# RazonIn4K/image-restoration-platform

Measured on AMD Instinct MI355X. Metric: restored images/sec @1024x1024 bs=8, higher is better.
Workload: dtype bf16; 1 GPU; 1024x1024 RGB u8, batch 8 per GPU: fused classifier scan + RestoreNet-v0 (43 convs, 779.9 GFLOP/image), seeded random-init weights; global_batch=8, parallelism=per-image data parallel x1, no collective, streams=1

## Files before the change

### image_restoration_platform_amd/csrc/conv_up.hip

```cpp
#include "conv_mfma.hpp"
#include "persist.hpp"

#include <type_traits>

namespace ire {

namespace {

typedef __bf16 bf16x8_t __attribute__((ext_vector_type(8)));
typedef __bf16 bf16x2_t __attribute__((ext_vector_type(2)));
typedef float f32x2_t __attribute__((ext_vector_type(2)));
typedef float f32x16_t __attribute__((ext_vector_type(16)));
typedef unsigned u32x4_t __attribute__((ext_vector_type(4)));

#ifndef IRE_UP_TEPI
#define IRE_UP_TEPI 1
#endif
#ifndef IRE_UP_ABL
#define IRE_UP_ABL 0
#endif
constexpr int UP_THREADS = 512;
constexpr int UP_TH = 16, UP_TW = 32;
constexpr int UP_IH = UP_TH + 2, UP_IW = UP_TW + 2;
constexpr int UP_IN_CHUNKS = UP_IH * UP_IW * 4;
constexpr int UP_IN_ITERS = (UP_IN_CHUNKS + UP_THREADS - 1) / UP_THREADS;
constexpr int UP_IN_BYTES = UP_IN_ITERS * UP_THREADS * 16;
constexpr int UP_NT = 32;
constexpr int UP_W_CHUNKS = 4 * 16 * UP_NT;
constexpr int UP_W_BYTES = UP_W_CHUNKS * 16;
constexpr int UP_W_ITERS = UP_W_CHUNKS / UP_THREADS;
constexpr int UP_BUF = UP_IN_BYTES + UP_W_BYTES;
constexpr int UP_BIAS_OFF = 2 * UP_BUF;
constexpr int UP_SKW_OFF = UP_BIAS_OFF + 256 * 4;
constexpr int UP_RED_OFF = UP_SKW_OFF + 8192;
constexpr int UP_LDS = UP_RED_OFF + 8 * 8 * 2 * 4;
static_assert(UP_LDS <= 160 * 1024, "LDS");
constexpr int UP_PATCH = UP_BUF / 8;

__device__ __forceinline__ unsigned up_pack(float a, float b) {
    f32x2_t f = {a, b};
    return __builtin_bit_cast(unsigned, __builtin_convertvector(f, bf16x2_t));
}
__device__ __forceinline__ void up_glds16(const void* gsrc, unsigned lds_dst_uniform) {
    unsigned keep;
    asm volatile("s_mov_b32 %0, m0\n\ts_mov_b32 m0, %2\n\ts_nop 0\n\tglobal_load_lds_dwordx4 %1, off\n\ts_mov_b32 m0, %0"
                 : "=&s"(keep) : "v"(gsrc), "s"(lds_dst_uniform) : "memory");
}

template <int N> __device__ __forceinline__ float up_ror_add(float v) {
    const int r = __builtin_amdgcn_update_dpp(0, __builtin_bit_cast(int, v), 0x120 + N, 0xf, 0xf, false);
    return v + __builtin_bit_cast(float, r);
}
__device__ __forceinline__ float up_swap16_add(float v) {
    float x = v, y = v;
    asm volatile("v_nop\n\tv_nop\n\tv_permlane16_swap_b32 %0, %1" : "+v"(x), "+v"(y));
    return x + y;
}

template <int I, int N, class F> __device__ __forceinline__ void up_static_for(F& f) {
    if constexpr (I < N) { f(std::integral_constant<int, I>{}); up_static_for<I + 1, N>(f); }
}

using UpItem = PersistItem;
struct UpRegs { uint4 v[UP_IN_ITERS]; };

template <int NKS>
__global__ __launch_bounds__(UP_THREADS) void conv_up_kernel(ConvArgs a) {
    __shared__ __attribute__((aligned(16))) unsigned char smem[UP_LDS];
    const unsigned smem_lds = (unsigned)(size_t)(__attribute__((address_space(3))) unsigned char*)smem;
    const int tid = threadIdx.x;
    const int lane = tid & 63, wave = tid >> 6;
    const int r = lane & 31, h = lane >> 5;
    const int c8_fixed = tid & 3;

    PersistCursor cursor(a.tiles_x, a.tiles_y, a.nimg, a.nblocks, a.nkc, (int)gridDim.x, (int)blockIdx.x, a.walk_rev != 0);
    const int my_items = cursor.my_items;
    const int nkc = a.nkc;
    const int S = cursor.S;
    if (S == 0) return;
    using StageInfo = PersistStage;
    StageInfo sq0 = cursor.cur, sq1 = cursor.next(), sq2 = cursor.next();

    const int Cin = a.cin0;
    const int cin_shift = 31 - __builtin_clz(Cin);

    int a_off[2][9];
#pragma unroll
    for (int m = 0; m < 2; ++m)
#pragma unroll
        for (int tap = 0; tap < 9; ++tap) {
            const int ky = tap / 3, kx = tap - ky * 3;
            const int p = (wave * 2 + m + ky) * UP_IW + r + kx;
            a_off[m][tap] = (p * 4 + (h ^ ((p >> 2) & 3))) * 16;
        }
    const int b_off = (h * UP_NT + r) * 16;

    auto load_chunk = [&](const StageInfo& si, int i, UpRegs& R) {
        const UpItem& it = si.it;
        const int oy1 = it.ty * UP_TH - 1, ox1 = it.tx * UP_TW - 1;
        const char* base = reinterpret_cast<const char*>(a.in0) + (size_t)it.img * a.in_rows * a.Win * Cin * 2 + si.kc * 64;
        const __amdgpu_buffer_rsrc_t irsrc = __builtin_amdgcn_make_buffer_rsrc(const_cast<char*>(base), 0, a.in_rows * a.Win * Cin * 2 - si.kc * 64, 0x00020000);
        int t2 = tid;
        asm volatile("" : "+v"(t2));
        const int p = (t2 + i * UP_THREADS) >> 2;
        const int py = p / UP_IW, px = p - py * UP_IW;
        const int iy = oy1 + py, ix = ox1 + px;
        const bool ok = (unsigned)(iy - a.iy_lo) < (unsigned)a.iy_span && (unsigned)ix < (unsigned)a.Win;
        const unsigned off = ok ? ((unsigned)((iy + a.in_row_off) * a.Win + ix) << (cin_shift + 1)) + (unsigned)(c8_fixed * 16) : 0xffffffffu;
        const u32x4_t lv = __builtin_amdgcn_raw_buffer_load_b128(irsrc, off, 0, 0);
        R.v[i] = make_uint4(lv.x, lv.y, lv.z, lv.w);
    };
    auto load_stage = [&](const StageInfo& si, UpRegs& R) {
#pragma unroll
        for (int i = 0; i < UP_IN_ITERS; ++i) load_chunk(si, i, R);
    };
    auto store_chunk = [&](int i, const UpRegs& R, uint4* lds_in) {
        int t2 = tid;
        asm volatile("" : "+v"(t2));
        const int idx = t2 + i * UP_THREADS;
        const int p = idx >> 2;
        lds_in[p * 4 + (c8_fixed ^ ((p >> 2) & 3))] = R.v[i];
    };
    auto wslab = [&](const StageInfo& si) -> const unsigned char* {
        return reinterpret_cast<const unsigned char*>(a.w) + ((size_t)si.it.nb * nkc + si.kc) * UP_W_BYTES;
    };

    f32x16_t acc[4][2];
    const float* bias_lds = reinterpret_cast<const float*>(smem + UP_BIAS_OFF);
    const int tiles_per_img = a.tiles_x * a.tiles_y;
    UpRegs R;

    auto epilogue = [&](const UpItem& it) __attribute__((always_inline)) {
        int r_e = r, h_e = h, w_e = wave;
        asm volatile("" : "+v"(r_e), "+v"(h_e), "+v"(w_e));
        char* obase = reinterpret_cast<char*>(a.out) + (size_t)it.img * a.Hout * a.Wout * a.cout * 2;
        const __amdgpu_buffer_rsrc_t orsrc = __builtin_amdgcn_make_buffer_rsrc(obase, 0, a.Hout * a.Wout * a.cout * 2, 0x00020000);
        const int ly = it.ty * UP_TH + w_e * 2, lx = it.tx * UP_TW + r_e;
        if constexpr (NKS > 0) {
            constexpr int NKG = NKS / 2;
            constexpr int U = 8 * NKG;
#ifdef IRE_UP_D
            constexpr int D = IRE_UP_D;
#else
            constexpr int D = NKS <= 2 ? 4 : NKS == 4 ? 3 : 2;
#endif
            const int C = a.cout;
            const char* sbase = reinterpret_cast<const char*>(a.in1) + (size_t)it.img * a.Hout * a.Wout * C * 2;
            const __amdgpu_buffer_rsrc_t srsrc = __builtin_amdgcn_make_buffer_rsrc(const_cast<char*>(sbase), 0, a.Hout * a.Wout * C * 2, 0x00020000);
            const unsigned rowB = (unsigned)(a.Wout * C * 2), pxB = (unsigned)(C * 2);
            const unsigned s_off = (unsigned)((2 * ly) * a.Wout + 2 * lx) * pxB + (unsigned)(h_e * 16);
            const bool inb[2] = {ly < a.Hin && lx < a.Win, ly + 1 < a.Hin && lx < a.Win};
            const unsigned char* skw = smem + UP_SKW_OFF + (h_e * 32 + r_e) * 16;
            const bf16x2_t ones = __builtin_bit_cast(bf16x2_t, 0x3f803f80u);
            u32x4_t ring[D][2];
            float ssum[4] = {0.f, 0.f, 0.f, 0.f}, qsum[4] = {0.f, 0.f, 0.f, 0.f};
            auto issue = [&](auto u_tag) __attribute__((always_inline)) {
                constexpr int u = decltype(u_tag)::value;
                constexpr int pm = u / NKG, kg = u % NKG, par = pm >> 1, m = pm & 1, pa = par >> 1, pb = par & 1;
                const unsigned off = s_off + (unsigned)(2 * m + pa) * rowB + (unsigned)pb * pxB + (unsigned)(kg * 64);
                ring[u % D][0] = __builtin_amdgcn_raw_buffer_load_b128(srsrc, off, 0, 0);
                ring[u % D][1] = __builtin_amdgcn_raw_buffer_load_b128(srsrc, off + 32u, 0, 0);
            };
            auto consume = [&](auto u_tag) __attribute__((always_inline)) {
                constexpr int u = decltype(u_tag)::value;
                constexpr int pm = u / NKG, kg = u % NKG, par = pm >> 1, m = pm & 1;
                const bf16x8_t w0 = __builtin_bit_cast(bf16x8_t, *reinterpret_cast<const uint4*>(skw + (2 * kg) * 1024));
                const bf16x8_t w1 = __builtin_bit_cast(bf16x8_t, *reinterpret_cast<const uint4*>(skw + (2 * kg + 1) * 1024));
                acc[par][m] = __builtin_amdgcn_mfma_f32_32x32x16_bf16(w0, __builtin_bit_cast(bf16x8_t, ring[u % D][0]), acc[par][m], 0, 0, 0);
                acc[par][m] = __builtin_amdgcn_mfma_f32_32x32x16_bf16(w1, __builtin_bit_cast(bf16x8_t, ring[u % D][1]), acc[par][m], 0, 0, 0);
            };
            auto finish = [&](auto par_tag) __attribute__((always_inline)) {
                constexpr int par = decltype(par_tag)::value;
                constexpr int pa = par >> 1, pb = par & 1;
                const int ox = 2 * lx + pb;
#pragma unroll
                for (int m = 0; m < 2; ++m) {
                    const int oy = 2 * (ly + m) + pa;
                    const unsigned off = ((unsigned)((oy * a.Wout + ox) * a.cout + it.nb * UP_NT) << 1) + (unsigned)(h_e * 16);
                    const f32x16_t& c = acc[par][m];
#pragma unroll
                    for (int pp = 0; pp < 2; ++pp) {
                        unsigned w[4] = {up_pack(c[8 * pp + 0], c[8 * pp + 1]), up_pack(c[8 * pp + 2], c[8 * pp + 3]),
                                         up_pack(c[8 * pp + 4], c[8 * pp + 5]), up_pack(c[8 * pp + 6], c[8 * pp + 7])};
                        const u32x4_t wv4 = {w[0], w[1], w[2], w[3]};
                        if constexpr (!(IRE_UP_ABL & 4)) __builtin_amdgcn_raw_buffer_store_b128(wv4, orsrc, inb[m] ? off + (unsigned)(pp * 32) : 0xffffffffu, 0, IRE_ST_PART);
                        else asm volatile("" :: "v"(wv4));
                        if constexpr (!(IRE_UP_ABL & 2))
#pragma unroll
                        for (int d = 0; d < 4; ++d) {
                            const bf16x2_t wv = __builtin_bit_cast(bf16x2_t, inb[m] ? w[d] : 0u);
                            ssum[2 * pp + (d >> 1)] = __builtin_amdgcn_fdot2_f32_bf16(wv, ones, ssum[2 * pp + (d >> 1)], false);
                            qsum[2 * pp + (d >> 1)] = __builtin_amdgcn_fdot2_f32_bf16(wv, wv, qsum[2 * pp + (d >> 1)], false);
                        }
                    }
                }
            };
            auto unit = [&](auto u_tag) __attribute__((always_inline)) {
                constexpr int u = decltype(u_tag)::value;
                if constexpr (!(IRE_UP_ABL & 1)) {
                consume(u_tag);
                if constexpr (u + D < U) issue(std::integral_constant<int, u + D>{});
                }
                if constexpr ((u + 1) % (2 * NKG) == 0) finish(std::integral_constant<int, u / (2 * NKG)>{});
            };
            if constexpr (!(IRE_UP_ABL & 1)) up_static_for<0, D>(issue);
            up_static_for<0, U>(unit);
            if constexpr (!(IRE_UP_ABL & 2)) {
            float rv[8] = {ssum[0], qsum[0], ssum[1], qsum[1], ssum[2], qsum[2], ssum[3], qsum[3]};
#pragma unroll
            for (int i = 0; i < 8; ++i) rv[i] = up_ror_add<1>(rv[i]);
#pragma unroll
            for (int i = 0; i < 8; ++i) rv[i] = up_ror_add<2>(rv[i]);
#pragma unroll
            for (int i = 0; i < 8; ++i) rv[i] = up_ror_add<4>(rv[i]);
#pragma unroll
            for (int i = 0; i < 8; ++i) rv[i] = up_ror_add<8>(rv[i]);
#pragma unroll
            for (int i = 0; i < 8; ++i) rv[i] = up_swap16_add(rv[i]);
            float* red = reinterpret_cast<float*>(smem + UP_RED_OFF);
            if (r_e == 0) {
#pragma unroll
                for (int k = 0; k < 4; ++k)
                    *reinterpret_cast<float2*>(red + (w_e * 8 + (k >> 1) * 4 + 2 * h_e + (k & 1)) * 2) = make_float2(rv[2 * k], rv[2 * k + 1]);
            }
            __syncthreads();
            const int G = a.group_size, qpg = G >> 2, ngl = UP_NT / G;
            if (tid < ngl) {
                float sv = 0.f, qv = 0.f;
#pragma unroll
                for (int w = 0; w < 8; ++w)
#pragma unroll
                    for (int k = 0; k < 4; ++k)
                        if (k < qpg) { sv += red[(w * 8 + tid * qpg + k) * 2 + 0]; qv += red[(w * 8 + tid * qpg + k) * 2 + 1]; }
                float* st = a.stats + (((size_t)it.img * tiles_per_img + it.tile) * 8 + (it.nb * UP_NT) / G + tid) * 2;
                st[0] = sv; st[1] = qv;
            }
            }
        } else {
#pragma unroll
        for (int par = 0; par < 4; ++par) {
            const int pa = par >> 1, pb = par & 1;
            const int ox = 2 * lx + pb;
#pragma unroll
            for (int m = 0; m < 2; ++m) {
                const int oy = 2 * (ly + m) + pa;
                const bool inb = oy < a.Hout && ox < a.Wout;
                const unsigned off = ((unsigned)((oy * a.Wout + ox) * a.cout + it.nb * UP_NT) << 1) + (unsigned)(h_e * 16);
                const f32x16_t& c = acc[par][m];
#pragma unroll
                for (int pp = 0; pp < 2; ++pp) {
                    const u32x4_t wv4 = {up_pack(c[8 * pp + 0], c[8 * pp + 1]), up_pack(c[8 * pp + 2], c[8 * pp + 3]),
                                         up_pack(c[8 * pp + 4], c[8 * pp + 5]), up_pack(c[8 * pp + 6], c[8 * pp + 7])};
                    __builtin_amdgcn_raw_buffer_store_b128(wv4, orsrc, inb ? off + (unsigned)(pp * 32) : 0xffffffffu, 0, IRE_ST_PART);
                }
            }
        }
        }
#pragma unroll
        for (int par = 0; par < 4; ++par)
#pragma unroll
            for (int m = 0; m < 2; ++m) asm volatile("" : "=v"(acc[par][m]));
    };

    u32x4_t skpre[4];
    auto epi_prefetch = [&](const UpItem& it) __attribute__((always_inline)) {
        constexpr int C = 16 * (NKS > 0 ? NKS : 2);
        int l_e = lane, w_e = wave;
        asm volatile("" : "+v"(l_e), "+v"(w_e));
        const char* sbase = reinterpret_cast<const char*>(a.in1) + (size_t)it.img * a.Hout * a.Wout * C * 2;
        const __amdgpu_buffer_rsrc_t srsrc = __builtin_amdgcn_make_buffer_rsrc(const_cast<char*>(sbase), 0, a.Hout * a.Wout * C * 2, 0x00020000);
        const int ly = it.ty * UP_TH + w_e * 2, ox0 = 2 * it.tx * UP_TW;
        const int lc = l_e & 3, lp0 = l_e >> 2;
        const bool rowok = ly < a.Hin;
#pragma unroll
        for (int i = 0; i < 4; ++i) {
            const int p = lp0 + i * 16;
            const bool ok = rowok && ox0 + p < a.Wout;
            skpre[i] = __builtin_amdgcn_raw_buffer_load_b128(srsrc, ok ? (unsigned)((((2 * ly) * a.Wout + ox0 + p) * C + lc * 8) * 2) : 0xffffffffu, 0, C == 32 ? IRE_LD_ONCE : 0);
        }
    };
    auto epilogue_t = [&](const UpItem& it) __attribute__((always_inline)) {
        constexpr int C = 16 * (NKS > 0 ? NKS : 2);
        constexpr int PCH = 32;
        constexpr int NPIECE = C / PCH;
        constexpr int CPP = PCH / 8;
        constexpr int KSP = PCH / 16;
        constexpr int PSTEP = 64 / CPP;
        int l_e = lane, w_e = wave;
        asm volatile("" : "+v"(l_e), "+v"(w_e));
        const int r_e = l_e & 31, h_e = l_e >> 5;
        unsigned char* patch = smem + UP_BUF + w_e * UP_PATCH;
        char* obase = reinterpret_cast<char*>(a.out) + (size_t)it.img * a.Hout * a.Wout * C * 2;
        const __amdgpu_buffer_rsrc_t orsrc = __builtin_amdgcn_make_buffer_rsrc(obase, 0, a.Hout * a.Wout * C * 2, 0x00020000);
        const char* sbase = reinterpret_cast<const char*>(a.in1) + (size_t)it.img * a.Hout * a.Wout * C * 2;
        const __amdgpu_buffer_rsrc_t srsrc = __builtin_amdgcn_make_buffer_rsrc(const_cast<char*>(sbase), 0, a.Hout * a.Wout * C * 2, 0x00020000);
        const int ly = it.ty * UP_TH + w_e * 2, ox0 = 2 * it.tx * UP_TW;
        const unsigned char* skw = smem + UP_SKW_OFF + (h_e * 32 + r_e) * 16;
        const bf16x2_t ones = __builtin_bit_cast(bf16x2_t, 0x3f803f80u);
        const int lc = l_e % CPP, lp0 = l_e / CPP;
        const unsigned ld_lds = (unsigned)(lp0 * (CPP * 16) + ((lc ^ ((lp0 >> 1) & (CPP - 1))) << 4));
        const int sp0 = l_e >> 2, scq = l_e & 3;
        float ssum[2] = {0.f, 0.f}, qsum[2] = {0.f, 0.f};
        u32x4_t sk[CPP];
        auto issue_piece = [&](int rr, int pc) __attribute__((always_inline)) {
            const int m = rr >> 1, pa = rr & 1;
            const int oy = 2 * (ly + m) + pa;
            const bool rowok = ly + m < a.Hin;
#pragma unroll
            for (int i = 0; i < CPP; ++i) {
                const int p = lp0 + i * PSTEP;
                const bool ok = rowok && ox0 + p < a.Wout;
                sk[i] = __builtin_amdgcn_raw_buffer_load_b128(srsrc, ok ? (unsigned)(((oy * a.Wout + ox0 + p) * C + pc * PCH + lc * 8) * 2) : 0xffffffffu, 0, C == 32 ? IRE_LD_ONCE : 0);
            }
        };
        if constexpr (!(IRE_UP_ABL & 1)) {
#pragma unroll
            for (int i = 0; i < CPP; ++i) sk[i] = skpre[i];
        }
#pragma unroll
        for (int rr = 0; rr < 4; ++rr) {
            const int m = rr >> 1, pa = rr & 1;
            if constexpr (!(IRE_UP_ABL & 1))
#pragma unroll
            for (int pc = 0; pc < NPIECE; ++pc) {
#pragma unroll
                for (int i = 0; i < CPP; ++i) *reinterpret_cast<u32x4_t*>(patch + ld_lds + i * (PSTEP * CPP * 16)) = sk[i];
                if (rr * NPIECE + pc + 1 < 4 * NPIECE) issue_piece((rr * NPIECE + pc + 1) / NPIECE, (rr * NPIECE + pc + 1) % NPIECE);
#pragma unroll
                for (int pb = 0; pb < 2; ++pb)
#pragma unroll
                    for (int k = 0; k < KSP; ++k) {
                        const bf16x8_t wk = __builtin_bit_cast(bf16x8_t, *reinterpret_cast<const uint4*>(skw + (pc * KSP + k) * 1024));
                        const bf16x8_t fr = __builtin_bit_cast(bf16x8_t, *reinterpret_cast<const uint4*>(patch + (2 * r_e + pb) * (CPP * 16) + (((2 * k + h_e) ^ (r_e & (CPP - 1))) << 4)));
                        acc[pa * 2 + pb][m] = __builtin_amdgcn_mfma_f32_32x32x16_bf16(wk, fr, acc[pa * 2 + pb][m], 0, 0, 0);
                    }
            }
            const int oy = 2 * (ly + m) + pa;
            const bool rowok = ly + m < a.Hin;
#pragma unroll
            for (int pb = 0; pb < 2; ++pb) {
                const f32x16_t& c = acc[pa * 2 + pb][m];
#pragma unroll
                for (int pp = 0; pp < 2; ++pp) {
                    const u32x4_t wv = {up_pack(c[8 * pp + 0], c[8 * pp + 1]), up_pack(c[8 * pp + 2], c[8 * pp + 3]),
                                        up_pack(c[8 * pp + 4], c[8 * pp + 5]), up_pack(c[8 * pp + 6], c[8 * pp + 7])};
                    *reinterpret_cast<u32x4_t*>(patch + (2 * r_e + pb) * 64 + (((2 * pp + h_e) ^ (r_e & 3)) << 4)) = wv;
                }
            }
#pragma unroll
            for (int k = 0; k < 4; ++k) {
                const int p = sp0 + 16 * k;
                const u32x4_t v = *reinterpret_cast<const u32x4_t*>(patch + p * 64 + ((scq ^ ((p >> 1) & 3)) << 4));
                const bool ok = rowok && ox0 + p < a.Wout;
                const unsigned w[4] = {v.x, v.y, v.z, v.w};
                if constexpr (!(IRE_UP_ABL & 2))
#pragma unroll
                for (int d = 0; d < 4; ++d) {
                    const bf16x2_t bv = __builtin_bit_cast(bf16x2_t, ok ? w[d] : 0u);
                    ssum[d >> 1] = __builtin_amdgcn_fdot2_f32_bf16(bv, ones, ssum[d >> 1], false);
                    qsum[d >> 1] = __builtin_amdgcn_fdot2_f32_bf16(bv, bv, qsum[d >> 1], false);
                }
                if constexpr (!(IRE_UP_ABL & 4)) __builtin_amdgcn_raw_buffer_store_b128(v, orsrc, ok ? (unsigned)(((oy * a.Wout + ox0 + p) * C + it.nb * UP_NT + scq * 8) * 2) : 0xffffffffu, 0, (C == 32 ? IRE_ST_LINE : IRE_ST_PART));
                else asm volatile("" :: "v"(v));
            }
        }
        if constexpr (!(IRE_UP_ABL & 2)) {
            float rv[4] = {ssum[0], qsum[0], ssum[1], qsum[1]};
#pragma unroll
            for (int i = 0; i < 4; ++i) rv[i] = up_ror_add<4>(rv[i]);
#pragma unroll
            for (int i = 0; i < 4; ++i) rv[i] = up_ror_add<8>(rv[i]);
#pragma unroll
            for (int i = 0; i < 4; ++i) rv[i] = up_swap16_add(rv[i]);
#pragma unroll
            for (int i = 0; i < 4; ++i) { float x = rv[i], y = rv[i]; asm volatile("v_nop\n\tv_nop\n\tv_permlane32_swap_b32 %0, %1" : "+v"(x), "+v"(y)); rv[i] = x + y; }
            float* red = reinterpret_cast<float*>(smem + UP_RED_OFF);
            if (l_e < 4) {
                *reinterpret_cast<float2*>(red + (w_e * 8 + 2 * l_e) * 2) = make_float2(rv[0], rv[1]);
                *reinterpret_cast<float2*>(red + (w_e * 8 + 2 * l_e + 1) * 2) = make_float2(rv[2], rv[3]);
            }
            __syncthreads();
            const int G = a.group_size, qpg = G >> 2, ngl = UP_NT / G;
            if (tid < ngl) {
                float sv = 0.f, qv = 0.f;
#pragma unroll
                for (int w = 0; w < 8; ++w)
#pragma unroll
                    for (int k = 0; k < 4; ++k)
                        if (k < qpg) { sv += red[(w * 8 + tid * qpg + k) * 2 + 0]; qv += red[(w * 8 + tid * qpg + k) * 2 + 1]; }
                float* st = a.stats + (((size_t)it.img * tiles_per_img + it.tile) * 8 + (it.nb * UP_NT) / G + tid) * 2;
                st[0] = sv; st[1] = qv;
            }
        } else __syncthreads();
#pragma unroll
        for (int par = 0; par < 4; ++par)
#pragma unroll
            for (int m = 0; m < 2; ++m) asm volatile("" : "=v"(acc[par][m]));
    };

    auto init_acc = [&](int nb) {
        const float* bl = bias_lds + nb * UP_NT + 8 * h;
#pragma unroll
        for (int q = 0; q < 4; ++q) {
            const float4 bv = *reinterpret_cast<const float4*>(bl + 16 * (q >> 1) + 4 * (q & 1));
#pragma unroll
            for (int par = 0; par < 4; ++par)
#pragma unroll
                for (int m = 0; m < 2; ++m) { acc[par][m][4 * q + 0] = bv.x; acc[par][m][4 * q + 1] = bv.y; acc[par][m][4 * q + 2] = bv.z; acc[par][m][4 * q + 3] = bv.w; }
        }
    };
    auto stage = [&](int s, auto par_tag, auto last_tag) {
        constexpr int PAR = decltype(par_tag)::value;
        constexpr int LASTV = decltype(last_tag)::value;
        constexpr bool LAST = LASTV == 1, PRELAST = LASTV == 2;
        const unsigned char* ib = smem + PAR * UP_BUF;
        uint4* in_nxt = reinterpret_cast<uint4*>(smem + (PAR ^ 1) * UP_BUF);
        const unsigned char* wb = smem + PAR * UP_BUF + UP_IN_BYTES + b_off;
        unsigned char* w_nxt = smem + (PAR ^ 1) * UP_BUF + UP_IN_BYTES;
#pragma unroll
        for (int i = 0; i < UP_IN_ITERS; ++i) asm volatile("" : "+v"(R.v[i].x), "+v"(R.v[i].y), "+v"(R.v[i].z), "+v"(R.v[i].w));
        bf16x8_t afr[2][2], bfr[2][4];
        auto read_group = [&](auto g_tag, bf16x8_t (&af)[2], bf16x8_t (&bf)[4]) __attribute__((always_inline)) {
            constexpr int g = decltype(g_tag)::value;
            constexpr int tap = g >> 1, cp = g & 1, ky = tap / 3, kx = tap - ky * 3;
#pragma unroll
            for (int m = 0; m < 2; ++m)
                af[m] = __builtin_bit_cast(bf16x8_t, *reinterpret_cast<const uint4*>(ib + (a_off[m][tap] ^ (cp << 5))));
            int n = 0;
#pragma unroll
            for (int pa = 0; pa < 2; ++pa)
#pragma unroll
                for (int pb = 0; pb < 2; ++pb) {
                    const int dy = ky - pa, dx = kx - pb;
                    if (dy < 0 || dy > 1 || dx < 0 || dx > 1) continue;
                    const int par = pa * 2 + pb, tap4 = dy * 2 + dx;
                    bf[n++] = __builtin_bit_cast(bf16x8_t, *reinterpret_cast<const uint4*>(wb + ((par * 16 + tap4 * 4 + 2 * cp) * UP_NT) * 16));
                }
        };
        auto mfma_group = [&](auto g_tag, const bf16x8_t (&af)[2], const bf16x8_t (&bf)[4]) __attribute__((always_inline)) {
            constexpr int g = decltype(g_tag)::value;
            constexpr int tap = g >> 1, ky = tap / 3, kx = tap - ky * 3;
            int n = 0;
#pragma unroll
            for (int pa = 0; pa < 2; ++pa)
#pragma unroll
                for (int pb = 0; pb < 2; ++pb) {
                    const int dy = ky - pa, dx = kx - pb;
                    if (dy < 0 || dy > 1 || dx < 0 || dx > 1) continue;
                    const int par = pa * 2 + pb;
#pragma unroll
                    for (int m = 0; m < 2; ++m) acc[par][m] = __builtin_amdgcn_mfma_f32_32x32x16_bf16(bf[n], af[m], acc[par][m], 0, 0, 0);
                    ++n;
                }
        };
        constexpr bool PREFETCH = NKS > 0 && NKS <= 4 && LAST && (IRE_UP_ABL & 8);
        unsigned pf_off = 0, pf_lim = 0, pf_dummy = 0;
        const char* pf_base = nullptr;
        if constexpr (PREFETCH) {
            const int C = a.cout;
            pf_base = reinterpret_cast<const char*>(a.in1) + (size_t)sq0.it.img * a.Hout * a.Wout * C * 2;
            pf_off = (unsigned)((2 * (sq0.it.ty * UP_TH + wave * 2)) * a.Wout + 2 * (sq0.it.tx * UP_TW + r)) * (unsigned)(C * 2) + (unsigned)(h * 32);
            pf_lim = (unsigned)(a.Hout * a.Wout * C * 2 - 4);
        }
        auto group = [&](auto g_tag) __attribute__((always_inline)) {
            constexpr int g = decltype(g_tag)::value;
            if constexpr (PREFETCH && g < 4 * NKS) {
                constexpr int NKG = NKS / 2, pm = g / NKG, kg = g % NKG, par = pm >> 1, m = pm & 1, pa = par >> 1, pb = par & 1;
                unsigned off = pf_off + (unsigned)(2 * m + pa) * (unsigned)(a.Wout * a.cout * 2) + (unsigned)(pb * a.cout * 2) + (unsigned)(kg * 64);
                off = off < pf_lim ? off : pf_lim;
                asm volatile("global_load_dword %0, %1, %2" : "+v"(pf_dummy) : "v"(off), "s"(pf_base) : "memory");
            }
            if constexpr (g + 1 < 18) read_group(std::integral_constant<int, g + 1>{}, afr[(g + 1) & 1], bfr[(g + 1) & 1]);
            __builtin_amdgcn_sched_barrier(0);
            mfma_group(g_tag, afr[g & 1], bfr[g & 1]);
            if constexpr (g < UP_IN_ITERS) { store_chunk(g, R, in_nxt); load_chunk(sq2, g, R); }
            if constexpr (g == 0) {
                const unsigned char* ws = wslab(sq1);
                const int wave_u = __builtin_amdgcn_readfirstlane(wave);
                const unsigned w_nxt_lds = smem_lds + (unsigned)(w_nxt - smem);
#pragma unroll
                for (int i = 0; i < UP_W_ITERS; ++i) {
                    const int cbase = i * UP_THREADS + wave_u * 64;
                    up_glds16(ws + (size_t)(cbase + lane) * 16, w_nxt_lds + cbase * 16);
                }
            }
            if constexpr (NKS > 0 && PRELAST && g == 1) {
                const int wave_u = __builtin_amdgcn_readfirstlane(wave);
                if (wave_u < NKS)
                    up_glds16(reinterpret_cast<const unsigned char*>(a.w1) + ((size_t)sq0.it.nb * NKS + wave_u) * 1024 + lane * 16,
                              smem_lds + UP_SKW_OFF + wave_u * 1024);
            }
            __builtin_amdgcn_sched_barrier(0);
        };
        read_group(std::integral_constant<int, 0>{}, afr[0], bfr[0]);
        group(std::integral_constant<int, 0>{}); group(std::integral_constant<int, 1>{}); group(std::integral_constant<int, 2>{});
        group(std::integral_constant<int, 3>{}); group(std::integral_constant<int, 4>{}); group(std::integral_constant<int, 5>{});
        group(std::integral_constant<int, 6>{}); group(std::integral_constant<int, 7>{}); group(std::integral_constant<int, 8>{});
        group(std::integral_constant<int, 9>{}); group(std::integral_constant<int, 10>{}); group(std::integral_constant<int, 11>{});
        group(std::integral_constant<int, 12>{}); group(std::integral_constant<int, 13>{}); group(std::integral_constant<int, 14>{});
        group(std::integral_constant<int, 15>{}); group(std::integral_constant<int, 16>{}); group(std::integral_constant<int, 17>{});
        asm volatile("s_waitcnt vmcnt(0)" ::: "memory");
        if constexpr (PREFETCH) asm volatile("" :: "v"(pf_dummy));
        if constexpr (LAST && NKS > 0 && IRE_UP_TEPI) {
            if constexpr (!(IRE_UP_ABL & 1)) epi_prefetch(sq0.it);
            __syncthreads();
            epilogue_t(sq0.it);
        } else {
            if constexpr (LAST) epilogue(sq0.it);
            __syncthreads();
        }
        sq0 = sq1; sq1 = sq2; sq2 = cursor.next();
    };

    {
        float* bl = reinterpret_cast<float*>(smem + UP_BIAS_OFF);
        if (tid < a.cout && tid < 256) bl[tid] = a.bias[tid];
        load_stage(sq0, R);
        const uint4* ws = reinterpret_cast<const uint4*>(wslab(sq0));
        uint4* wd = reinterpret_cast<uint4*>(smem + UP_IN_BYTES);
        for (int i = tid; i < UP_W_CHUNKS; i += UP_THREADS) wd[i] = ws[i];
        uint4* in0 = reinterpret_cast<uint4*>(smem);
#pragma unroll
        for (int i = 0; i < UP_IN_ITERS; ++i) store_chunk(i, R, in0);
        load_stage(sq1, R);
    }
    __syncthreads();
    int s = 0;
    for (int k = 0; k < my_items; ++k) {
        init_acc(sq0.it.nb);
        for (int kc = 0; kc + 2 < nkc; kc += 2) {
            stage(s, std::integral_constant<int, 0>{}, std::integral_constant<int, 0>{}); ++s;
            stage(s, std::integral_constant<int, 1>{}, std::integral_constant<int, 0>{}); ++s;
        }
        stage(s, std::integral_constant<int, 0>{}, std::integral_constant<int, 2>{}); ++s;
        stage(s, std::integral_constant<int, 1>{}, std::integral_constant<int, 1>{}); ++s;
    }
    asm volatile("s_waitcnt vmcnt(0)" ::: "memory");
}

}

void conv_up_subpixel_launch(const ConvArgs& a, hipStream_t stream) {
    if (a.nkc < 2 || (a.nkc & 1) || a.cout > 256) fail(IRE_ERR_INTERNAL, "internal: conv_up_subpixel shape");
    if (a.in1 && (!a.w1 || !a.stats || (a.cout != 32 && a.cout != 64 && a.cout != 128))) fail(IRE_ERR_INTERNAL, "internal: fused conv_up arguments");
    const int items = a.tiles_x * a.tiles_y * a.nimg * a.nblocks;
    const int cus = persistent_grid_cus();
    const int grid = items < cus ? items : cus;
    if (!a.in1) hipLaunchKernelGGL(conv_up_kernel<0>, dim3(grid), dim3(UP_THREADS), 0, stream, a);
    else if (a.cout == 32) hipLaunchKernelGGL(conv_up_kernel<2>, dim3(grid), dim3(UP_THREADS), 0, stream, a);
    else if (a.cout == 64) hipLaunchKernelGGL(conv_up_kernel<4>, dim3(grid), dim3(UP_THREADS), 0, stream, a);
    else hipLaunchKernelGGL(conv_up_kernel<8>, dim3(grid), dim3(UP_THREADS), 0, stream, a);
    IRE_HIP(hipGetLastError());
}

}
```

Baseline: 1093 images/sec.

## Defer next-stage input loads into fused epilogue and ring-buffer skip prefetch

In the last k-chunk stage of the fused upsampling conv, the global loads for the next stage's input tile are moved out of the MFMA loop and spread across the epilogue's skip-piece loop. This is meant to hide their latency behind epilogue work and to relieve memory pressure during the MFMA phase. The skip-tensor prefetch becomes a configurable ring of register buffers, defaulting to 2 pieces, replacing the single prefetched piece. The A-operand LDS offsets are now recomputed per item under an asm barrier, which trades a few ALU ops for lower register pressure. The added in-flight registers could raise VGPR use and lower occupancy.

```diff
diff --git a/image_restoration_platform_amd/csrc/conv_up.hip b/image_restoration_platform_amd/csrc/conv_up.hip
--- a/image_restoration_platform_amd/csrc/conv_up.hip
+++ b/image_restoration_platform_amd/csrc/conv_up.hip
@@ -36,6 +36,13 @@
 constexpr int UP_LDS = UP_RED_OFF + 8 * 8 * 2 * 4;
 static_assert(UP_LDS <= 160 * 1024, "LDS");
 constexpr int UP_PATCH = UP_BUF / 8;
+constexpr int UP_PCH = 32, UP_CPP = UP_PCH / 8, UP_PSTEP = 64 / UP_CPP;
+#ifdef IRE_UP_RING
+template <int NKS> constexpr int up_ring() { return IRE_UP_RING < 2 * (NKS > 0 ? NKS : 2) ? IRE_UP_RING : 2 * (NKS > 0 ? NKS : 2); }
+#else
+template <int NKS> constexpr int up_ring() { return 2; }
+#endif
+static_assert(64 * UP_CPP * 16 <= UP_PATCH, "skip piece");
 
 __device__ __forceinline__ unsigned up_pack(float a, float b) {
     f32x2_t f = {a, b};
@@ -85,14 +92,18 @@
     const int cin_shift = 31 - __builtin_clz(Cin);
 
     int a_off[2][9];
-#pragma unroll
-    for (int m = 0; m < 2; ++m)
-#pragma unroll
-        for (int tap = 0; tap < 9; ++tap) {
-            const int ky = tap / 3, kx = tap - ky * 3;
-            const int p = (wave * 2 + m + ky) * UP_IW + r + kx;
-            a_off[m][tap] = (p * 4 + (h ^ ((p >> 2) & 3))) * 16;
-        }
+    auto set_a_off = [&]() __attribute__((always_inline)) {
+        int r_a = r, h_a = h, w_a = wave;
+        asm volatile("" : "+v"(r_a), "+v"(h_a), "+v"(w_a));
+#pragma unroll
+        for (int m = 0; m < 2; ++m)
+#pragma unroll
+            for (int tap = 0; tap < 9; ++tap) {
+                const int ky = tap / 3, kx = tap - ky * 3;
+                const int p = (w_a * 2 + m + ky) * UP_IW + r_a + kx;
+                a_off[m][tap] = (p * 4 + (h_a ^ ((p >> 2) & 3))) * 16;
+            }
+    };
     const int b_off = (h * UP_NT + r) * 16;
 
     auto load_chunk = [&](const StageInfo& si, int i, UpRegs& R) {
@@ -262,30 +273,37 @@
             for (int m = 0; m < 2; ++m) asm volatile("" : "=v"(acc[par][m]));
     };
 
-    u32x4_t skpre[4];
+    constexpr int RING = up_ring<NKS>();
+    u32x4_t sk[RING][UP_CPP];
     auto epi_prefetch = [&](const UpItem& it) __attribute__((always_inline)) {
-        constexpr int C = 16 * (NKS > 0 ? NKS : 2);
+        constexpr int C = 16 * (NKS > 0 ? NKS : 2), NPIECE = C / UP_PCH;
         int l_e = lane, w_e = wave;
         asm volatile("" : "+v"(l_e), "+v"(w_e));
         const char* sbase = reinterpret_cast<const char*>(a.in1) + (size_t)it.img * a.Hout * a.Wout * C * 2;
         const __amdgpu_buffer_rsrc_t srsrc = __builtin_amdgcn_make_buffer_rsrc(const_cast<char*>(sbase), 0, a.Hout * a.Wout * C * 2, 0x00020000);
         const int ly = it.ty * UP_TH + w_e * 2, ox0 = 2 * it.tx * UP_TW;
-        const int lc = l_e & 3, lp0 = l_e >> 2;
-        const bool rowok = ly < a.Hin;
-#pragma unroll
-        for (int i = 0; i < 4; ++i) {
-            const int p = lp0 + i * 16;
-            const bool ok = rowok && ox0 + p < a.Wout;
-            skpre[i] = __builtin_amdgcn_raw_buffer_load_b128(srsrc, ok ? (unsigned)((((2 * ly) * a.Wout + ox0 + p) * C + lc * 8) * 2) : 0xffffffffu, 0, C == 32 ? IRE_LD_ONCE : 0);
+        const int lc = l_e % UP_CPP, lp0 = l_e / UP_CPP;
+#pragma unroll
+        for (int q = 0; q < RING; ++q) {
+            const int rr = q / NPIECE, pc = q % NPIECE, m = rr >> 1, pa = rr & 1;
+            const int oy = 2 * (ly + m) + pa;
+            const unsigned rowout = ~(unsigned)((ly + m - a.Hin) >> 31);
+#pragma unroll
+            for (int i = 0; i < UP_CPP; ++i) {
+                const int p = lp0 + i * UP_PSTEP;
+                const unsigned out = rowout | ~(unsigned)((ox0 + p - a.Wout) >> 31);
+                sk[q][i] = __builtin_amdgcn_raw_buffer_load_b128(srsrc, (unsigned)(((oy * a.Wout + ox0 + p) * C + pc * UP_PCH + lc * 8) * 2) | out, 0, C == 32 ? IRE_LD_ONCE : 0);
+            }
         }
     };
     auto epilogue_t = [&](const UpItem& it) __attribute__((always_inline)) {
         constexpr int C = 16 * (NKS > 0 ? NKS : 2);
-        constexpr int PCH = 32;
+        constexpr int PCH = UP_PCH;
         constexpr int NPIECE = C / PCH;
-        constexpr int CPP = PCH / 8;
+        constexpr int CPP = UP_CPP;
         constexpr int KSP = PCH / 16;
-        constexpr int PSTEP = 64 / CPP;
+        constexpr int PSTEP = UP_PSTEP;
+        constexpr int NP = 4 * NPIECE;
         int l_e = lane, w_e = wave;
         asm volatile("" : "+v"(l_e), "+v"(w_e));
         const int r_e = l_e & 31, h_e = l_e >> 5;
@@ -301,31 +319,38 @@
         const unsigned ld_lds = (unsigned)(lp0 * (CPP * 16) + ((lc ^ ((lp0 >> 1) & (CPP - 1))) << 4));
         const int sp0 = l_e >> 2, scq = l_e & 3;
         float ssum[2] = {0.f, 0.f}, qsum[2] = {0.f, 0.f};
-        u32x4_t sk[CPP];
-        auto issue_piece = [&](int rr, int pc) __attribute__((always_inline)) {
+        auto r_landed = [&]() __attribute__((always_inline)) {
+#pragma unroll
+            for (int i = 0; i < UP_IN_ITERS; ++i) asm volatile("" : "+v"(R.v[i].x), "+v"(R.v[i].y), "+v"(R.v[i].z), "+v"(R.v[i].w));
+        };
+        if constexpr ((IRE_UP_ABL & 1) != 0) load_stage(sq2, R);
+        auto issue_piece = [&](int rr, int pc, u32x4_t (&dst)[CPP]) __attribute__((always_inline)) {
             const int m = rr >> 1, pa = rr & 1;
             const int oy = 2 * (ly + m) + pa;
-            const bool rowok = ly + m < a.Hin;
+            const unsigned rowout = ~(unsigned)((ly + m - a.Hin) >> 31);
 #pragma unroll
             for (int i = 0; i < CPP; ++i) {
                 const int p = lp0 + i * PSTEP;
-                const bool ok = rowok && ox0 + p < a.Wout;
-                sk[i] = __builtin_amdgcn_raw_buffer_load_b128(srsrc, ok ? (unsigned)(((oy * a.Wout + ox0 + p) * C + pc * PCH + lc * 8) * 2) : 0xffffffffu, 0, C == 32 ? IRE_LD_ONCE : 0);
+                const unsigned out = rowout | ~(unsigned)((ox0 + p - a.Wout) >> 31);
+                dst[i] = __builtin_amdgcn_raw_buffer_load_b128(srsrc, (unsigned)(((oy * a.Wout + ox0 + p) * C + pc * PCH + lc * 8) * 2) | out, 0, C == 32 ? IRE_LD_ONCE : 0);
             }
         };
-        if constexpr (!(IRE_UP_ABL & 1)) {
-#pragma unroll
-            for (int i = 0; i < CPP; ++i) sk[i] = skpre[i];
-        }
 #pragma unroll
         for (int rr = 0; rr < 4; ++rr) {
             const int m = rr >> 1, pa = rr & 1;
             if constexpr (!(IRE_UP_ABL & 1))
 #pragma unroll
             for (int pc = 0; pc < NPIECE; ++pc) {
-#pragma unroll
-                for (int i = 0; i < CPP; ++i) *reinterpret_cast<u32x4_t*>(patch + ld_lds + i * (PSTEP * CPP * 16)) = sk[i];
-                if (rr * NPIECE + pc + 1 < 4 * NPIECE) issue_piece((rr * NPIECE + pc + 1) / NPIECE, (rr * NPIECE + pc + 1) % NPIECE);
+                const int q = rr * NPIECE + pc;
+#pragma unroll
+                for (int i = 0; i < CPP; ++i) *reinterpret_cast<u32x4_t*>(patch + ld_lds + i * (PSTEP * CPP * 16)) = sk[q % RING][i];
+                if (q + RING < NP) issue_piece((q + RING) / NPIECE, (q + RING) % NPIECE, sk[q % RING]);
+                else {
+                    const int j = q + RING - NP;
+#pragma unroll
+                    for (int i = 0; i < UP_IN_ITERS; ++i)
+                        if (i >= 4 * j && (i < 4 * (j + 1) || j == RING - 1)) load_chunk(sq2, i, R);
+                }
 #pragma unroll
                 for (int pb = 0; pb < 2; ++pb)
 #pragma unroll
@@ -379,6 +404,7 @@
                 *reinterpret_cast<float2*>(red + (w_e * 8 + 2 * l_e) * 2) = make_float2(rv[0], rv[1]);
                 *reinterpret_cast<float2*>(red + (w_e * 8 + 2 * l_e + 1) * 2) = make_float2(rv[2], rv[3]);
             }
+            r_landed();
             __syncthreads();
             const int G = a.group_size, qpg = G >> 2, ngl = UP_NT / G;
             if (tid < ngl) {
@@ -391,7 +417,7 @@
                 float* st = a.stats + (((size_t)it.img * tiles_per_img + it.tile) * 8 + (it.nb * UP_NT) / G + tid) * 2;
                 st[0] = sv; st[1] = qv;
             }
-        } else __syncthreads();
+        } else { r_landed(); __syncthreads(); }
 #pragma unroll
         for (int par = 0; par < 4; ++par)
 #pragma unroll
@@ -417,8 +443,6 @@
         uint4* in_nxt = reinterpret_cast<uint4*>(smem + (PAR ^ 1) * UP_BUF);
         const unsigned char* wb = smem + PAR * UP_BUF + UP_IN_BYTES + b_off;
         unsigned char* w_nxt = smem + (PAR ^ 1) * UP_BUF + UP_IN_BYTES;
-#pragma unroll
-        for (int i = 0; i < UP_IN_ITERS; ++i) asm volatile("" : "+v"(R.v[i].x), "+v"(R.v[i].y), "+v"(R.v[i].z), "+v"(R.v[i].w));
         bf16x8_t afr[2][2], bfr[2][4];
         auto read_group = [&](auto g_tag, bf16x8_t (&af)[2], bf16x8_t (&bf)[4]) __attribute__((always_inline)) {
             constexpr int g = decltype(g_tag)::value;
@@ -473,7 +497,7 @@
             if constexpr (g + 1 < 18) read_group(std::integral_constant<int, g + 1>{}, afr[(g + 1) & 1], bfr[(g + 1) & 1]);
             __builtin_amdgcn_sched_barrier(0);
             mfma_group(g_tag, afr[g & 1], bfr[g & 1]);
-            if constexpr (g < UP_IN_ITERS) { store_chunk(g, R, in_nxt); load_chunk(sq2, g, R); }
+            if constexpr (g < UP_IN_ITERS) { store_chunk(g, R, in_nxt); if constexpr (!(LAST && NKS > 0 && IRE_UP_TEPI)) load_chunk(sq2, g, R); }
             if constexpr (g == 0) {
                 const unsigned char* ws = wslab(sq1);
                 const int wave_u = __builtin_amdgcn_readfirstlane(wave);
@@ -500,6 +524,8 @@
         group(std::integral_constant<int, 12>{}); group(std::integral_constant<int, 13>{}); group(std::integral_constant<int, 14>{});
         group(std::integral_constant<int, 15>{}); group(std::integral_constant<int, 16>{}); group(std::integral_constant<int, 17>{});
         asm volatile("s_waitcnt vmcnt(0)" ::: "memory");
+#pragma unroll
+        for (int i = 0; i < UP_IN_ITERS; ++i) asm volatile("" : "+v"(R.v[i].x), "+v"(R.v[i].y), "+v"(R.v[i].z), "+v"(R.v[i].w));
         if constexpr (PREFETCH) asm volatile("" :: "v"(pf_dummy));
         if constexpr (LAST && NKS > 0 && IRE_UP_TEPI) {
             if constexpr (!(IRE_UP_ABL & 1)) epi_prefetch(sq0.it);
@@ -523,10 +549,13 @@
 #pragma unroll
         for (int i = 0; i < UP_IN_ITERS; ++i) store_chunk(i, R, in0);
         load_stage(sq1, R);
+#pragma unroll
+        for (int i = 0; i < UP_IN_ITERS; ++i) asm volatile("" : "+v"(R.v[i].x), "+v"(R.v[i].y), "+v"(R.v[i].z), "+v"(R.v[i].w));
     }
     __syncthreads();
     int s = 0;
     for (int k = 0; k < my_items; ++k) {
+        set_a_off();
         init_acc(sq0.it.nb);
         for (int kc = 0; kc + 2 < nkc; kc += 2) {
             stage(s, std::integral_constant<int, 0>{}, std::integral_constant<int, 0>{}); ++s;
```

Measured after the change: 1094 images/sec, median of 6. Within noise of the previous version (+0.1%).
